# Onetism/LightFieldMicroscopy_PC-bzip2

Measured on AMD Instinct MI355X. Metric: uint16 Mpixel/s encode (predictor->bzip2) at 1/2/4/8 GPUs; ratio parity, higher is better.
Workload: dtype u16

## Files before the change

### lightfieldmicroscopy_pc-bzip2_amd/csrc/lfm_bzip2.hip

```cpp
#include <hip/hip_runtime.h>
#include <rocprim/block/block_exchange.hpp>
#include <rocprim/block/block_sort.hpp>
#include <rocprim/device/device_radix_sort.hpp>
#include <rocprim/device/device_scan.hpp>
#include <rocprim/device/device_segmented_radix_sort.hpp>
#include <rocprim/device/device_select.hpp>
#include <rocprim/iterator/counting_iterator.hpp>
#include <algorithm>
#include <climits>
#include <cstdlib>
#include <cstdint>
#include <cstdio>
#include <cstring>
#include <mutex>
#include <type_traits>
#include <vector>
#include "lfm_bwt_types.h"
#include "lfm_bz_caps.h"
#include "lfm_hip.h"
#include "lfm_huff_heap.h"

#ifndef LFM_BWT_FORCE_FULL
#define LFM_BWT_FORCE_FULL 0
#endif

namespace lfm {
namespace bz {

constexpr int kRleThreads = 512;
constexpr int kMaxGroups = 6;
constexpr int kMaxAlpha = 258;
constexpr int kIters = 4;
constexpr uint32_t kRunA = 0, kRunB = 1;

constexpr uint32_t kFlagHost = 1;

struct Geometry {
    uint32_t dims[5];
    uint32_t bs[5];
    uint32_t nb[5];
    uint32_t bpp;
};

struct Batch {
    const uint8_t* img;
    Geometry g;
    uint32_t first_block;
    uint32_t nstreams;
    uint32_t raw_cap;
    uint32_t cap;
    uint32_t level;
    uint32_t nblock_max;
    uint32_t out_cap;
    uint8_t* raw;
    uint32_t* raw_len;
    uint8_t* T;
    uint32_t* n;
    uint32_t* crc;
    uint32_t* inuse;
    uint32_t* flags;
    uint32_t* done;
    uint64_t* keys_a;
    uint64_t* keys_b;
    uint32_t* vals_a;
    uint32_t* sa;
    uint32_t* rank;
    uint32_t* vals_b;
    uint32_t* cl0;
    uint32_t* cl1;
    uint8_t* uflag;
    uint32_t* seg_begin;
    uint32_t* seg_end;
    uint16_t* mtfv;
// ... 2390 lines not shown
                pos += nz ? 1u : 0u;
                z = nz ? 0u : z + 1u;
            }
        }
        {
            uint32_t dsum = 0;
            for (uint64_t r = R; r; r &= r - 1ull) {
                const uint32_t i = (uint32_t)__builtin_ctzll(r), z = run_len(i);
                digits(wr + (uint32_t)__popcll(NZ & ((1ull << i) - 1ull)) + dsum, z);
                dsum += run_digits(z);
            }
        }
        if (has_last) {
            if (zend) digits(wr + w - 1u - dend, zend);
            tile_out[rle2_swz(wr + w - 1u)] = (uint16_t)EOB;
            atomicAdd(&freq[EOB], 1u);
        }
        __syncthreads();
        const uint32_t base = s_wr;
        for (uint32_t i = t; i < tile_total; i += kRle2Threads) out[base + i] = tile_out[rle2_swz(i)];
        __syncthreads();
        if (t == 0) {
            s_wr = base + tile_total;
            s_carry = tile_end_zeros;
        }
        __syncthreads();
    }
    static_assert(kRunA == 0 && kRunB == 1, "RUNA / RUNB are symbols 0 and 1");
    uint32_t cnts[6] = {nrunA, nrunB, (uint32_t)(hot & 0xFFFFu), (uint32_t)((hot >> 16) & 0xFFFFu),
                        (uint32_t)((hot >> 32) & 0xFFFFu), (uint32_t)(hot >> 48)};
#pragma unroll
    for (int r = 0; r < 6; ++r) {
        uint32_t c = cnts[r];
        for (int d = 32; d > 0; d >>= 1) c += (uint32_t)__shfl_xor((int)c, d);
        if (lane == 0 && c) atomicAdd(&freq[r], c);
    }
    __syncthreads();
    if (t == 0) {
        B.nmtf[s] = s_wr;
        if (!heap_narrow(B, s, (int)nin + 2)) B.wide[atomicAdd(B.wide_cnt, 1u)] = s;
    }
    for (uint32_t v = t; v < kMaxAlpha; v += kRle2Threads) B.mtf_freq[(size_t)s * kMaxAlpha + v] = freq[v];
}

constexpr int kHuffThreads = 256;

__device__ __forceinline__ uint32_t stream_nin(const Batch& B, uint32_t s)
{
    uint32_t nin = 0;
    for (int q = 0; q < 8; ++q) nin += __popc(B.inuse[s * 8 + q]);
    return nin;
}

__global__ __launch_bounds__(64) void huff_init(Batch B)
{
    __shared__ int mf[kMaxAlpha];
    __shared__ int pgs[kMaxGroups], pge[kMaxGroups];
    const uint32_t s = blockIdx.x, t = threadIdx.x;
    if (B.flags[s] & kFlagHost) return;
    const uint32_t nMTF = B.nmtf[s];
    const int alphaSize = (int)stream_nin(B, s) + 2;
    const uint32_t* mfreq = B.mtf_freq + (size_t)s * kMaxAlpha;
    uint8_t* len = B.len + (size_t)s * kMaxGroups * kMaxAlpha;
    const int nGroups = nMTF < 200 ? 2 : nMTF < 600 ? 3 : nMTF < 1200 ? 4 : nMTF < 2400 ? 5 : 6;
    for (int v = t; v < kMaxAlpha; v += 64) mf[v] = v < alphaSize ? (int)mfreq[v] : 0;
    __syncthreads();
    if (t == 0) {
        int nPart = nGroups, remF = (int)nMTF, gs = 0;
        while (nPart > 0) {
            const int tFreq = remF / nPart;
            int ge = gs - 1, aFreq = 0;
            while (aFreq < tFreq && ge < alphaSize - 1) {
                ++ge;
                aFreq += mf[ge];
            }
            if (ge > gs && nPart != nGroups && nPart != 1 && ((nGroups - nPart) % 2 == 1)) {
                aFreq -= mf[ge];
                --ge;
            }
            pgs[nPart - 1] = gs;
            pge[nPart - 1] = ge;
            --nPart;
            gs = ge + 1;
            remF -= aFreq;
        }
        B.ngroups[s] = (uint32_t)nGroups;
        B.nsel[s] = (nMTF + kGSize - 1) / kGSize;
    }
    __syncthreads();
    for (int i = t; i < kMaxGroups * kMaxAlpha; i += 64) {
        const int q = i / kMaxAlpha, v = i - q * kMaxAlpha;
        len[i] = (q < nGroups && v < alphaSize && v >= pgs[q] && v <= pge[q]) ? 0 : 15;
    }
}

__global__ __launch_bounds__(kHuffThreads) void huff_select_reg(Batch B)
{
    __shared__ uint32_t rfreq[kMaxGroups][kMaxAlpha];
    __shared__ uint64_t lpack[kMaxAlpha + 1];
    __shared__ uint32_t junk[kHuffThreads];
    const uint32_t s = blockIdx.x, t = threadIdx.x;
    if (B.flags[s] & kFlagHost) return;
    const uint32_t nMTF = B.nmtf[s], nSel = B.nsel[s];
    const int nGroups = (int)B.ngroups[s];
    const int alphaSize = (int)stream_nin(B, s) + 2;
    const uint8_t* len = B.len + (size_t)s * kMaxGroups * kMaxAlpha;
    const uint16_t* mtfv = B.mtfv + (size_t)s * (B.cap + 8);
    uint8_t* sel = B.sel + (size_t)s * B.sel_cap;
    for (int i = t; i < kMaxGroups * kMaxAlpha; i += kHuffThreads) rfreq[i / kMaxAlpha][i % kMaxAlpha] = 0;
    for (int v = t; v <= kMaxAlpha; v += kHuffThreads) {
        uint64_t lp = 0;
        if (v < alphaSize)
            for (int q = 0; q < nGroups; ++q) lp |= (uint64_t)len[q * kMaxAlpha + v] << (10 * q);
        lpack[v] = lp;
    }
    __syncthreads();
    uint64_t lp_hot[4];
#pragma unroll
    for (int f = 0; f < 4; ++f) lp_hot[f] = lpack[f];
    for (uint32_t g = t; g < nSel; g += kHuffThreads) {
        const uint32_t gs = g * kGSize, cnt = min(nMTF - gs, (uint32_t)kGSize);
        uint32_t w[kGSize / 2];
        if (cnt == (uint32_t)kGSize) {
            const uint32_t* p = (const uint32_t*)(mtfv + gs);
#pragma unroll
            for (int q = 0; q < kGSize / 2; ++q) w[q] = p[q];
        } else {
#pragma unroll
            for (int q = 0; q < kGSize / 2; ++q) {
                const uint32_t lo = 2u * q < cnt ? mtfv[gs + 2 * q] : (uint32_t)kMaxAlpha;
                const uint32_t hi = 2u * q + 1 < cnt ? mtfv[gs + 2 * q + 1] : (uint32_t)kMaxAlpha;
                w[q] = lo | (hi << 16);
            }
        }
        uint32_t hot = 0;
        uint64_t acc = 0;
#pragma unroll
        for (int q = 0; q < kGSize / 2; ++q) {
            const uint32_t lo = w[q] & 0xFFFFu, hi = w[q] >> 16;
            hot += lo < 4u ? 1u << (8u * lo) : 0u;
            hot += hi < 4u ? 1u << (8u * hi) : 0u;
            acc += lpack[lo < 4u ? (uint32_t)kMaxAlpha : lo] + lpack[hi < 4u ? (uint32_t)kMaxAlpha : hi];
        }
#pragma unroll
        for (uint32_t f = 0; f < 4; ++f) acc += (uint64_t)((hot >> (8u * f)) & 0xFFu) * lp_hot[f];
        int bt = -1;
        uint32_t bc = 999999999u;
        for (int q = 0; q < nGroups; ++q) {
            const uint32_t cq = (uint32_t)(acc >> (10 * q)) & 1023u;
            if (cq < bc) { bc = cq; bt = q; }
        }
        sel[g] = (uint8_t)bt;
#pragma unroll
        for (int q = 0; q < kGSize / 2; ++q) {
            const uint32_t lo = w[q] & 0xFFFFu, hi = w[q] >> 16;
            atomicAdd(lo >= 4u && lo != (uint32_t)kMaxAlpha ? &rfreq[bt][lo] : &junk[t], 1u);
            atomicAdd(hi >= 4u && hi != (uint32_t)kMaxAlpha ? &rfreq[bt][hi] : &junk[t], 1u);
        }
#pragma unroll
        for (uint32_t f = 0; f < 4; ++f)
            if ((hot >> (8u * f)) & 0xFFu) atomicAdd(&rfreq[bt][f], (hot >> (8u * f)) & 0xFFu);
    }
    __syncthreads();
    uint32_t* rf = B.rfreq + (size_t)s * kMaxGroups * kMaxAlpha;
    for (int i = t; i < kMaxGroups * kMaxAlpha; i += kHuffThreads) rf[i] = rfreq[i / kMaxAlpha][i % kMaxAlpha];
}

template <typename Ent, int kL>
struct LdsHeap {
    static constexpr uint32_t RS = sizeof(Ent) * kL;
    char* base;
    uint16_t* parent;
    __device__ __forceinline__ Ent ld(uint32_t e) const { return *(const Ent*)(base + e * RS); }
    __device__ __forceinline__ void st(uint32_t e, Ent v) const { *(Ent*)(base + e * RS) = v; }
    __device__ __forceinline__ void ld_pair(uint32_t e, Ent& a, Ent& b) const
    {
        const char* q = base + e * RS;
        a = *(const Ent*)q;
        b = *(const Ent*)(q + RS);
    }
    __device__ __forceinline__ void fence() const { __builtin_amdgcn_sched_barrier(0); }
    __device__ __forceinline__ void set_parent(uint32_t node, uint32_t p) const { parent[node] = (uint16_t)p; }
    __device__ __forceinline__ bool any(bool b) const { return __builtin_amdgcn_ballot_w64(b) != 0; }
    __device__ __forceinline__ void note_sift(uint32_t, uint32_t) const {}
    __device__ __forceinline__ void note_push(uint32_t, uint32_t) const {}
    __device__ __forceinline__ void check(const HeapPref&, uint32_t) const {}
};

template <typename Ent>
constexpr int kHeapMaxRetries = sizeof(Ent) == 4 ? 17 : 32;

template <typename Ent, int kL>
__device__ __forceinline__ void heap_code_lengths(const Batch& B, char* hb, uint32_t lane, uint32_t s, uint32_t tb)
{
    constexpr uint32_t ES = sizeof(Ent);
    static_assert(kHeapEntries * sizeof(Ent) * kL <= 33792, "the heaps' LDS grew");
    static_assert(kHeapEntries >= kMaxAlpha + 2 && 2 * kMaxAlpha / (int)(ES / 2) < kHeapEntries, "heap entries");
    {
        const int A = (int)stream_nin(B, s) + 2;
        const uint32_t* freq = B.rfreq + ((size_t)s * kMaxGroups + tb) * kMaxAlpha;
        uint8_t* len = B.len + ((size_t)s * kMaxGroups + tb) * kMaxAlpha;
        uint16_t* parent = (uint16_t*)(B.code + ((size_t)s * kMaxGroups + tb) * kMaxAlpha);
        LdsHeap<Ent, kL> acc{hb + lane * ES, parent};
        auto ent = [&](uint32_t e) -> Ent& { return *(Ent*)(acc.base + e * LdsHeap<Ent, kL>::RS); };
        auto dep = [&](uint32_t k) -> uint16_t& {
            return *(uint16_t*)((char*)&ent(k / (ES / 2)) + 2 * (k % (ES / 2)));
        };
        auto ld2 = [](const void* p, int i) { return *(const uint2*)((const uint32_t*)p + (i > 0 ? i : 0)); };
        constexpr Ent kSent = ~(Ent)0;
        auto upheap_init = [&](uint32_t z) {
            constexpr int D = 9;
            Ent v[D + 1];
#pragma unroll
            for (int j = 0; j <= D; ++j) v[j] = ent(z >> j);
            __builtin_amdgcn_sched_barrier(0);
            const Ent k = v[0], kk = k | (Ent)1023;
            bool below = true;
#pragma unroll
            for (int j = 0; j < D; ++j) {
                const bool lt = kk < v[j + 1];
                ent(z >> j) = lt ? v[j + 1] : (below || j == 0 ? k : v[j]);
                below = lt;
            }
        };
        int retries = 0;
        uint32_t nMerged = (uint32_t)A;
        bool build = true;
        for (int round = 0; round <= kHeapMaxRetries<Ent>; ++round) {
            uint32_t nHeap = 1, tooLong = 0;
            Ent top = 0;
            HeapPref m;
            if (build) {
                ent(0) = 0;
                for (int e = A + 1; e < kHeapEntries; ++e) ent((uint32_t)e) = kSent;
                for (int i0 = 1; i0 <= A; i0 += 32) {
                    uint2 f[16];
#pragma unroll
                    for (int q = 0; q < 16; ++q) f[q] = ld2(freq, min(i0 - 1 + 2 * q, kMaxAlpha - 2));
#pragma unroll
                    for (int q = 0; q < 16; ++q) {
                        const int i = i0 + 2 * q;
                        uint32_t w0 = f[q].x ? f[q].x : 1u, w1 = f[q].y ? f[q].y : 1u;
                        for (int r = 0; r < retries; ++r) {
                            w0 = 1u + w0 / 2u;
                            w1 = 1u + w1 / 2u;
                        }
                        if (i <= A) ent(i) = ((Ent)w0 << 15) | (Ent)i;
                        if (i + 1 <= A) ent(i + 1) = ((Ent)w1 << 15) | (Ent)(i + 1);
                    }
                }
                for (int i = 1; i <= A; ++i) upheap_init((uint32_t)i);
                heap_pref_build<Ent>(acc, m, (uint32_t)A);
                nHeap = (uint32_t)A;
                nMerged = (uint32_t)A;
                top = ent(1);
            }
            uint32_t hmax = 0;
            for (int b = 8; b >= 0; --b) {
                const uint32_t a = build ? (uint32_t)A : 0u;
                if (__builtin_amdgcn_ballot_w64((a >> b & 1u) && (a >> (b + 1)) == (hmax >> (b + 1)))) hmax |= 1u << b;
            }
            hmax = min(__builtin_amdgcn_readfirstlane(hmax), (uint32_t)kMaxAlpha);
            for (; hmax > 1u; --hmax)
                if (build && nHeap > 1u) heap_merge_step_at<Ent>(acc, m, hmax, nHeap, nMerged, top, tooLong);
            build = build && tooLong && retries < kHeapMaxRetries<Ent>;
            if (build) ++retries;
            if (!__builtin_amdgcn_ballot_w64(build)) break;
        }
        const int nNodes = (int)nMerged;
        if (retries) atomicAdd(B.wide_cnt + 1, (uint32_t)retries);
        dep(nNodes) = 0;
        for (int kc = (nNodes - 1) & ~63; kc >= 0; kc -= 64) {
            uint2 pw[16];
#pragma unroll
            for (int q = 0; q < 16; ++q) pw[q] = ld2(parent, min(kc / 2 + 2 * q, (2 * kMaxAlpha) / 2 - 2));
#pragma unroll
            for (int q = 15; q >= 0; --q) {
                const int b = kc + 4 * q;
                const uint32_t p4[4] = {pw[q].x & 0xFFFFu, pw[q].x >> 16, pw[q].y & 0xFFFFu, pw[q].y >> 16};
                uint32_t d[4], dn[4];
#pragma unroll
                for (int r = 0; r < 4; ++r) d[r] = dep(min(p4[r], 2u * kMaxAlpha));
#pragma unroll
                for (int r = 3; r >= 0; --r) {
                    const int k = b + r;
                    uint32_t x = d[r];
#pragma unroll
                    for (int u = r + 1; u < 4; ++u) x = p4[r] == (uint32_t)(b + u) ? dn[u] : x;
                    dn[r] = k == nNodes ? 0u : x + 1u;
                    if (k >= 1 && k < nNodes) dep(k) = (uint16_t)dn[r];
                }
            }
        }
        for (int i = 1; i <= A; ++i) len[i - 1] = (uint8_t)dep(i);
    }
}

template <int kL>
__global__ __launch_bounds__(64) void huff_lengths_heap(Batch B, uint32_t nwg_wide, uint32_t nwide_streams)
{
    __shared__ uint32_t hq[kHeapEntries * kL];
    char* hb = (char*)hq;
    const uint32_t lane = threadIdx.x;
    if (blockIdx.x >= nwg_wide) {
        const uint32_t task = (blockIdx.x - nwg_wide) * kL + lane;
        const uint32_t s = task / kMaxGroups, tb = task % kMaxGroups;
        if (lane >= (uint32_t)kL || s >= B.nstreams || (B.flags[s] & kFlagHost) || tb >= B.ngroups[s]) return;
        if (!heap_narrow(B, s, (int)stream_nin(B, s) + 2)) return;
        heap_code_lengths<uint32_t, kL>(B, hb, lane, s, tb);
    } else {
        constexpr int kW = kL / 2;
        const uint32_t i = blockIdx.x * kW + lane;
        if (lane >= (uint32_t)kW || i >= nwide_streams * kMaxGroups) return;
        const uint32_t s = B.wide[i / kMaxGroups], tb = i % kMaxGroups;
        if ((B.flags[s] & kFlagHost) || tb >= B.ngroups[s]) return;
        heap_code_lengths<uint64_t, kW>(B, hb, lane, s, tb);
    }
}

__global__ __launch_bounds__(64) void huff_final(Batch B)
{
    const uint32_t s = blockIdx.x, lane = threadIdx.x;
    if (B.flags[s] & kFlagHost) return;
    const uint32_t nGroups = B.ngroups[s];
    const uint32_t nSel = B.nsel[s];
    const uint32_t alphaSize = stream_nin(B, s) + 2;
    const uint8_t* len = B.len + (size_t)s * kMaxGroups * kMaxAlpha;
    {
        const uint8_t* sel = B.sel + (size_t)s * B.sel_cap;
        uint8_t* sm = B.sel_mtf + (size_t)s * B.sel_cap;
        uint32_t pos = 0x543210u;
        for (uint32_t i0 = 0; i0 < nSel; i0 += 64) {
            const uint32_t cnt = min(64u, nSel - i0);
            const uint32_t v = lane < cnt ? sel[i0 + lane] : 0u;
            uint32_t out = 0;
            for (uint32_t g = 0; g < cnt; ++g) {
                const uint32_t ll = __builtin_amdgcn_readlane(v, g);
                const uint32_t x = pos ^ (ll * 0x111111u);
                const uint32_t z = (x - 0x111111u) & ~x & 0x888888u;
                const uint32_t j = (uint32_t)__builtin_ctz(z) >> 2;
                const uint32_t m = (1u << (4 * (j + 1))) - 1u;
                pos = (pos & ~m) | (((pos << 4) | ll) & m);
                out = lane == g ? j : out;
            }
            if (lane < cnt) sm[i0 + lane] = (uint8_t)out;
        }
    }
    const uint64_t lt = (1ull << lane) - 1ull;
    for (uint32_t q = 0; q < nGroups; ++q) {
        const uint8_t* lq = len + q * kMaxAlpha;
        uint32_t* code = B.code + ((size_t)s * kMaxGroups + q) * kMaxAlpha;
        uint32_t L[5], c[5];
#pragma unroll
        for (int k = 0; k < 5; ++k) {
            const uint32_t i = 64 * k + lane;
            L[k] = i < alphaSize ? lq[i] : 0u;
            c[k] = 0;
        }
        uint32_t vec = 0;
        for (uint32_t nl = 1; nl <= 20; ++nl) {
            uint32_t before = 0;
#pragma unroll
            for (int k = 0; k < 5; ++k) {
                const uint64_t b = __ballot(L[k] == nl);
                if (L[k] == nl) c[k] = vec + before + (uint32_t)__popcll(b & lt);
                before += (uint32_t)__popcll(b);
            }
            vec = (vec + before) << 1;
        }
#pragma unroll
        for (int k = 0; k < 5; ++k) {
            const uint32_t i = 64 * k + lane;
            if (i < alphaSize) code[i] = c[k];
        }
    }
}

constexpr int kEmitThreads = 256;

__device__ __forceinline__ void put_bits_atomic(uint32_t* words, uint64_t pos, uint32_t nbits, uint32_t v)
{
    if (!nbits) return;
    const uint32_t w = (uint32_t)(pos >> 5), o = (uint32_t)(pos & 31);
    const uint64_t sh = ((uint64_t)v << (64 - nbits)) >> o;
    const uint32_t hi = (uint32_t)(sh >> 32), lo = (uint32_t)sh;
    if (hi) atomicOr(&words[w], hi);
    if (lo) atomicOr(&words[w + 1], lo);
}

constexpr uint32_t kSelLds = 8192;

constexpr uint32_t kHdrWords = 4096;

__device__ __forceinline__ void put_bits_hdr(uint32_t* hdr, uint32_t* words, uint64_t pos, uint32_t nbits, uint32_t v)
{
    if (!nbits) return;
    const uint32_t w = (uint32_t)(pos >> 5), o = (uint32_t)(pos & 31);
    const uint64_t sh = ((uint64_t)v << (64 - nbits)) >> o;
    const uint32_t hi = (uint32_t)(sh >> 32), lo = (uint32_t)sh;
    if (w + 1 < kHdrWords) {
        hdr[w] |= hi;
        hdr[w + 1] |= lo;
    } else {
        if (hi) atomicOr(&words[w], hi);
        if (lo) atomicOr(&words[w + 1], lo);
    }
}

__device__ __forceinline__ void put_bits_hdr_atomic(uint32_t* hdr, uint32_t* words, uint64_t pos, uint32_t nbits,
                                                    uint32_t v)
{
    if (!nbits) return;
    const uint32_t w = (uint32_t)(pos >> 5), o = (uint32_t)(pos & 31);
    const uint64_t sh = ((uint64_t)v << (64 - nbits)) >> o;
    const uint32_t hi = (uint32_t)(sh >> 32), lo = (uint32_t)sh;
    if (w + 1 < kHdrWords) {
        if (hi) atomicOr(&hdr[w], hi);
        if (lo) atomicOr(&hdr[w + 1], lo);
    } else {
        if (hi) atomicOr(&words[w], hi);
        if (lo) atomicOr(&words[w + 1], lo);
    }
}

__device__ __forceinline__ void put_bits64_hdr_atomic(uint32_t* hdr, uint32_t* words, uint64_t pos, uint32_t nbits,
                                                      uint64_t v)
{
    if (nbits > 32) {
// ... 825 lines not shown
extern "C" size_t lfm_hip_bzip2_workspace_bytes_multi(uint32_t nstreams, uint32_t block_bytes, uint32_t level)
{
    if (level < 1 || level > 9) return 0;
    Batch B{};
    Scratch S{};
    return layout(nullptr, nstreams, block_bytes, level, B, S);
}

extern "C" uint32_t lfm_hip_bzip2_max_count_multi(uint32_t block_bytes, uint32_t level)
{
    if (level < 1 || level > 9) return 0;
    Batch B{};
    Scratch S{};
    (void)layout(nullptr, 0, block_bytes, level, B, S);
    return (uint32_t)(((1ull << 32) - 1) / ((uint64_t)B.parts * B.cap));
}

extern "C" size_t lfm_hip_bzip2_out_cap(uint32_t block_bytes) { return out_cap(block_bytes); }

namespace {
int bzip2_blocks(const void* d_img, const uint32_t dims[5], const uint32_t bs[5], uint32_t bpp, uint32_t first,
                 const uint32_t streams, uint32_t level, void* d_ws, size_t ws_bytes, void* d_payload,
                 uint64_t* h_sizes, uint32_t* h_flags, void* stream_, bool multi)
{
    uint32_t count = streams;
    hipStream_t st = (hipStream_t)stream_;
    if (!d_img || !dims || !bs || !bpp || !count || level < 1 || level > 9 || !d_ws || !d_payload) return LFM_HIP_EINVAL;
    int dev = 0;
    (void)hipGetDevice(&dev);
    if (!crc_tables_on_device(dev)) return LFM_HIP_ERUNTIME;
    StageEvents& SE = t_stage;
    SE.valid = false;
    const bool timed = SE.ready(dev);
    auto mark = [&](int i) {
        if (timed) (void)hipEventRecord(SE.ev[i], st);
    };
    Batch B{};
    B.img = (const uint8_t*)d_img;
    uint32_t raw_cap = bpp;
    for (int d = 0; d < 5; ++d) {
        B.g.dims[d] = dims[d];
        B.g.bs[d] = bs[d];
        B.g.nb[d] = (uint32_t)((dims[d] + bs[d] - 1) / bs[d]);
        raw_cap *= bs[d];
    }
    B.g.bpp = bpp;
    B.first_block = first;
    B.level = level;
    B.nblock_max = 100000u * level - 19u;
    Scratch S{};
    if (ws_bytes < layout((uint8_t*)d_ws, streams, raw_cap, multi ? level : 0u, B, S)) return LFM_HIP_EINVAL;
    count = B.nstreams;
    if ((size_t)count * B.cap >= (1ull << 32)) return LFM_HIP_EINVAL;
    const bool parts = B.parts > 1;

    hipError_t e = hipSuccess;
    auto ok = [&]() { return (e = hipGetLastError()) == hipSuccess; };
    const bool from_img = ((uintptr_t)d_img & 15) == 0 && (bs[0] * bpp) % 16 == 0 && (dims[0] * bpp) % 16 == 0 &&
                          ((dims[0] % bs[0]) * bpp) % 16 == 0;
    mark(0);
    if (!from_img) hipLaunchKernelGGL(gather_blocks, dim3(64, streams), dim3(256), 0, st, B);
    if (!parts) {
        if (from_img) hipLaunchKernelGGL((rle1_crc<true, false>), dim3(count), dim3(kRleThreads), 0, st, B);
        else hipLaunchKernelGGL((rle1_crc<false, false>), dim3(count), dim3(kRleThreads), 0, st, B);
    } else {
        if (from_img) hipLaunchKernelGGL((rle1_crc<true, true>), dim3(streams), dim3(kRleThreads), 0, st, B);
        else hipLaunchKernelGGL((rle1_crc<false, true>), dim3(streams), dim3(kRleThreads), 0, st, B);
        hipLaunchKernelGGL(place_parts, dim3(16, count), dim3(256), 0, st, B);
    }
    if (!ok()) return LFM_HIP_ERUNTIME;
    mark(1);
    BwtStats bwt_stats;
    B.ent = (uint2*)B.keys_a;
    if (bwt_sort(B, S, st, &bwt_stats) != hipSuccess) return LFM_HIP_ERUNTIME;
    t_last_place = bwt_stats.place_path(B.it_full != 0);
    {
        const uint32_t v[12] = {bwt_stats.chunks[0], bwt_stats.chunks[1], bwt_stats.chunks[2], bwt_stats.chunks[3],
                                bwt_stats.first_ties, bwt_stats.left_runs, bwt_stats.text_rounds, bwt_stats.restarted,
                                bwt_stats.rank_form, bwt_stats.doubling_rounds, bwt_stats.flag_periodic, 0u};
        std::copy(v, v + 12, t_last_bwt);
        std::copy(bwt_stats.jobs, bwt_stats.jobs + 4, t_last_jobs);
    }
    if (!B.it_full) {
        const uint32_t chunks = (B.cap + kPlaceChunk - 1) / kPlaceChunk;
        if (t_last_place == 2)
            hipLaunchKernelGGL(bwt_place_sorted, dim3(8 * chunks * ((count + 7) / 8)), dim3(256), 0, st, B, chunks);
        hipLaunchKernelGGL(bwt_induce, dim3(count), dim3(64), 0, st, B);
        if (!ok()) return LFM_HIP_ERUNTIME;
    }
    mark(2);
    if (t_hook) t_hook(t_hook_ctx, 1);
    {
        const uint32_t nseg_max = (B.cap + kSeg - 1) / kSeg;
        int32_t* seg_last = (int32_t*)B.keys_a;
        const dim3 g((nseg_max + 3) / 4, count);
        if (B.it_full) hipLaunchKernelGGL(mtf_last<false>, g, dim3(256), 0, st, B, nseg_max, seg_last);
        else hipLaunchKernelGGL(mtf_last<true>, g, dim3(256), 0, st, B, nseg_max, seg_last);
        hipLaunchKernelGGL(mtf_prefix, dim3(count), dim3(256), 0, st, B, nseg_max, seg_last);
        hipLaunchKernelGGL(mtf_win, g, dim3(256), 0, st, B, nseg_max, (const int32_t*)seg_last);
        hipLaunchKernelGGL(rle2, dim3(count), dim3(kRle2Threads), 0, st, B);
    }
    uint32_t nwide = 0;
    if (!ok() || hipMemcpyAsync(&nwide, B.wide_cnt, 4, hipMemcpyDeviceToHost, st) != hipSuccess ||
        hipStreamSynchronize(st) != hipSuccess || nwide > count)
        return LFM_HIP_ERUNTIME;
    mark(3);
    if (t_hook) t_hook(t_hook_ctx, 2);
    hipLaunchKernelGGL(huff_init, dim3(count), dim3(64), 0, st, B);
    static thread_local struct TablesEvent {
        hipEvent_t ev = nullptr;
        int dev = -1;
        ~TablesEvent()
        {
            if (ev) (void)hipEventDestroy(ev);
        }
    } tables_ev;
    if (t_hook && tables_ev.dev != dev) {
        if (tables_ev.ev) (void)hipEventDestroy(tables_ev.ev);
        tables_ev.ev = nullptr;
        tables_ev.dev = -1;
        if (hipEventCreateWithFlags(&tables_ev.ev, hipEventDisableTiming) == hipSuccess) tables_ev.dev = dev;
    }
    hipEvent_t ev_tables = tables_ev.ev;
    for (int it = 0; it < kIters; ++it) {
        hipLaunchKernelGGL(huff_select_reg, dim3(count), dim3(kHuffThreads), 0, st, B);
        constexpr uint32_t kPlane = 32;
        const uint32_t nn = (count * kMaxGroups + kPlane - 1) / kPlane;
        const uint32_t nw = (nwide * kMaxGroups + kPlane / 2 - 1) / (kPlane / 2);
        hipLaunchKernelGGL(huff_lengths_heap<kPlane>, dim3(nn + nw), dim3(64), 0, st, B, nw, nwide);
    }
    hipLaunchKernelGGL(huff_final, dim3(count), dim3(64), 0, st, B);
    mark(4);
    const bool hook3 = t_hook && ev_tables && hipEventRecord(ev_tables, st) == hipSuccess;
    Batch J = B;
    if (!parts) {
        hipLaunchKernelGGL(emit_stream<false>, dim3(count), dim3(kEmitThreads), 0, st, B);
    } else {
        hipLaunchKernelGGL(emit_stream<true>, dim3(count), dim3(kEmitThreads), 0, st, B);
        hipLaunchKernelGGL(join_parts, dim3(streams), dim3(256), 0, st, B);
        J.words = B.jwords;
        J.out_cap = B.jcap;
        J.out_bytes = B.sbytes;
        J.flags = B.sflags;
    }
    hipLaunchKernelGGL(scan_offsets, dim3(1), dim3(1024), 0, st, J.out_bytes, streams, S.offs);
    hipLaunchKernelGGL(compact_streams, dim3(streams), dim3(256), 0, st, J, S.offs, (uint8_t*)d_payload);
    mark(5);
    if (!ok()) return LFM_HIP_ERUNTIME;
    if (hook3 && hipEventSynchronize(ev_tables) == hipSuccess) t_hook(t_hook_ctx, 3);
    static const bool stats = std::getenv("LFM_BZ2_STATS") && std::atoi(std::getenv("LFM_BZ2_STATS")) != 0;
    if (stats) {
        uint32_t c[8] = {};
        if (hipMemcpyAsync(c, S.cnt, 32, hipMemcpyDeviceToHost, st) == hipSuccess && hipStreamSynchronize(st) == hipSuccess)
            std::fprintf(stderr, "lfm_bzip2 stats: %u streams, %u with u64 Huffman heaps, Huffman retries %u, "
                         "tied after the chunk sorts %u, runs left to the tie rounds %u\n", count, c[3], c[4],
                         bwt_stats.first_ties, bwt_stats.left_runs);
    }
    std::vector<uint32_t> nbytes(streams), np(streams, 1u);
    if (hipMemcpyAsync(nbytes.data(), J.out_bytes, streams * 4, hipMemcpyDeviceToHost, st) != hipSuccess ||
        hipMemcpyAsync(h_flags, J.flags, streams * 4, hipMemcpyDeviceToHost, st) != hipSuccess ||
        (parts && hipMemcpyAsync(np.data(), B.nparts, streams * 4, hipMemcpyDeviceToHost, st) != hipSuccess) ||
        hipStreamSynchronize(st) != hipSuccess)
        return LFM_HIP_ERUNTIME;
    for (uint32_t i = 0; i < streams; ++i) h_sizes[i] = nbytes[i];
    t_last_blocks = 0;
    for (uint32_t i = 0; i < streams; ++i) t_last_blocks += h_flags[i] ? 0u : np[i];
    if (timed) {
        SE.valid = true;
        for (int i = 0; i < 5; ++i)
            if (hipEventElapsedTime(&SE.last_ms[i], SE.ev[i], SE.ev[i + 1]) != hipSuccess) SE.valid = false;
    }
    return LFM_HIP_OK;
}
}

extern "C" int lfm_hip_bzip2_blocks(const void* d_img, const uint32_t dims[5], const uint32_t bs[5], uint32_t bpp,
                                    uint32_t first, uint32_t count, uint32_t level, void* d_ws, size_t ws_bytes,
                                    void* d_payload, uint64_t* h_sizes, uint32_t* h_flags, void* stream)
{
    return bzip2_blocks(d_img, dims, bs, bpp, first, count, level, d_ws, ws_bytes, d_payload, h_sizes, h_flags, stream,
                        false);
}

extern "C" int lfm_hip_bzip2_blocks_multi(const void* d_img, const uint32_t dims[5], const uint32_t bs[5],
                                          uint32_t bpp, uint32_t first, uint32_t count, uint32_t level, void* d_ws,
                                          size_t ws_bytes, void* d_payload, uint64_t* h_sizes, uint32_t* h_flags,
                                          void* stream)
{
    return bzip2_blocks(d_img, dims, bs, bpp, first, count, level, d_ws, ws_bytes, d_payload, h_sizes, h_flags, stream,
                        true);
}

extern "C" void lfm_hip_bzip2_set_stage_hook(void (*fn)(void*, int), void* ctx)
{
    t_hook = fn;
    t_hook_ctx = ctx;
}

extern "C" uint64_t lfm_hip_bzip2_last_blocks(void) { return t_last_blocks; }

extern "C" void lfm_hip_bzip2_last_bwt_stats(uint32_t out[12])
{
    if (out) std::copy(t_last_bwt, t_last_bwt + 12, out);
}

extern "C" void lfm_hip_bzip2_last_sort_jobs(uint32_t out[4])
{
    if (out) std::copy(t_last_jobs, t_last_jobs + 4, out);
}

extern "C" uint32_t lfm_hip_bzip2_last_place_path(void) { return t_last_place; }

extern "C" int lfm_hip_bzip2_last_stage_ms(float ms[5])
{
    if (!ms || !t_stage.valid) return 3;
    for (int i = 0; i < 5; ++i) ms[i] = t_stage.last_ms[i];
    return 0;
}
```

### lightfieldmicroscopy_pc-bzip2_amd/csrc/lfm_huff_heap.h

```cpp
#pragma once
#include <cstdint>

#ifndef LFM_HD
#if defined(__HIPCC__) || defined(__CUDACC__)
#define LFM_HD __host__ __device__
#else
#define LFM_HD
#endif
#endif

constexpr int kHeapEntries = 264;
constexpr uint32_t kHeapSentPair = 260;
constexpr int kHeapMaxLevels = 8;
constexpr int kPrefWords = 5;

struct HeapPref {
    uint32_t w[kPrefWords];
};

template <typename Ent>
LFM_HD inline bool heap_wless(Ent a, Ent b)
{
    return (a | (Ent)1023) < b;
}

template <typename Ent>
LFM_HD inline Ent heap_sent()
{
    return ~(Ent)0;
}

LFM_HD inline uint32_t heap_pref_at(const HeapPref& m, int j, uint32_t p)
{
    if (j <= 4) return (m.w[0] >> (p & 31u)) & 1u;
    if (j == 5) return (m.w[1] >> (p & 31u)) & 1u;
    if (j == 6) return ((p & 32u ? m.w[3] : m.w[2]) >> (p & 31u)) & 1u;
    const uint32_t b = p - 128u < 31u ? p - 128u : 31u;
    return (m.w[4] >> b) & 1u;
}

LFM_HD inline uint32_t heap_put_bit(uint32_t w, uint32_t b, uint32_t bit)
{
    return (w & ~(1u << b)) | (bit << b);
}

LFM_HD inline void heap_pref_flip(HeapPref& d, int j, uint32_t p, uint32_t flip)
{
    if (j <= 4) {
        d.w[0] |= flip << (p & 31u);
    } else if (j == 5) {
        d.w[1] |= flip << (p & 31u);
    } else if (j == 6) {
        const uint32_t x = flip << (p & 31u);
        d.w[2] |= p & 32u ? 0u : x;
        d.w[3] |= p & 32u ? x : 0u;
    } else {
        const uint32_t b = p - 128u < 31u ? p - 128u : 31u;
        d.w[4] |= flip << b;
    }
}

LFM_HD inline void heap_pref_set_any(HeapPref& m, uint32_t p, uint32_t bit)
{
    const uint32_t b = p & 31u, wi = p >> 5;
#pragma unroll
    for (uint32_t i = 0; i < (uint32_t)kPrefWords; ++i) m.w[i] = wi == i ? heap_put_bit(m.w[i], b, bit) : m.w[i];
}

template <typename Ent, typename Acc>
LFM_HD inline void heap_pref_build(Acc& acc, HeapPref& m, uint32_t A)
{
    const uint32_t last = A >> 1;
#pragma unroll
    for (uint32_t wi = 0; wi < (uint32_t)kPrefWords; ++wi) {
        uint32_t word = 0;
        for (uint32_t b0 = 0; b0 < 32u && 32u * wi + b0 <= last; b0 += 8u) {
            Ent l[8], r[8];
#pragma unroll
            for (uint32_t q = 0; q < 8u; ++q) {
                const uint32_t p = 32u * wi + b0 + q;
                acc.ld_pair(2u * (p <= last ? p : last), l[q], r[q]);
            }
            acc.fence();
#pragma unroll
            for (uint32_t q = 0; q < 8u; ++q) {
                const uint32_t p = 32u * wi + b0 + q;
                word |= (p >= 1u && p <= last && heap_wless(r[q], l[q]) ? 1u : 0u) << (b0 + q);
            }
        }
        m.w[wi] = word;
    }
}

template <int L, typename Ent, typename Acc>
LFM_HD inline Ent heap_sift_path(Acc& acc, HeapPref& m, Ent k)
{
    if constexpr (L == 0) {
        acc.st(1u, k);
        acc.note_sift(0u, 0u);
        return k;
    } else {
        uint32_t p[L + 1], cb[L], r[L];
        p[0] = 1u;
#pragma unroll
        for (int j = 0; j < L; ++j) {
            r[j] = heap_pref_at(m, j, p[j]);
            cb[j] = 2u * p[j];
            if (j == 7) cb[j] = cb[j] < kHeapSentPair ? cb[j] : kHeapSentPair;
            p[j + 1] = cb[j] | r[j];
        }
        Ent a[L], b[L];
#pragma unroll
        for (int j = 0; j < L; ++j) acc.ld_pair(cb[j], a[j], b[j]);
        acc.fence();
        const Ent kk = k | (Ent)1023;
        Ent c[L], sib[L], nv[L + 1];
        bool go[L];
        bool g = true;
        uint32_t went = 0;
#pragma unroll
        for (int j = 0; j < L; ++j) {
// ... 135 lines not shown
```

Before: 19000.

## Parallelize selector MTF scan, fold huff_init into first select pass, split huff_final waves

Replaces the serial per-selector MTF loop in huff_final with a wave-wide parallel prefix scan over MTF-list summaries, and runs it in a dedicated wave alongside per-group code-assignment waves. huff_init is removed, and its partitioning is folded into a templated first huff_select_reg pass, which saves a launch and a global round-trip of the length table. Heap initial build is restructured into level-templated inserts, and optional timestamp instrumentation is added. This adds composition work per lane and requires 16-byte alignment of selector buffers.

```diff
diff --git a/lightfieldmicroscopy_pc-bzip2_amd/csrc/lfm_bzip2.hip b/lightfieldmicroscopy_pc-bzip2_amd/csrc/lfm_bzip2.hip
--- a/lightfieldmicroscopy_pc-bzip2_amd/csrc/lfm_bzip2.hip
+++ b/lightfieldmicroscopy_pc-bzip2_amd/csrc/lfm_bzip2.hip
@@ -19,6 +19,7 @@
 #include "lfm_bz_caps.h"
 #include "lfm_hip.h"
 #include "lfm_huff_heap.h"
+#include "lfm_sel_mtf.h"
 
 #ifndef LFM_BWT_FORCE_FULL
 #define LFM_BWT_FORCE_FULL 0
@@ -2515,18 +2516,11 @@
     return nin;
 }
 
-__global__ __launch_bounds__(64) void huff_init(Batch B)
-{
-    __shared__ int mf[kMaxAlpha];
-    __shared__ int pgs[kMaxGroups], pge[kMaxGroups];
-    const uint32_t s = blockIdx.x, t = threadIdx.x;
-    if (B.flags[s] & kFlagHost) return;
-    const uint32_t nMTF = B.nmtf[s];
-    const int alphaSize = (int)stream_nin(B, s) + 2;
+__device__ __forceinline__ void huff_partition(const Batch& B, uint32_t s, uint32_t t, uint32_t nthreads, uint32_t nMTF,
+                                               int alphaSize, int nGroups, int* mf, int* pgs, int* pge)
+{
     const uint32_t* mfreq = B.mtf_freq + (size_t)s * kMaxAlpha;
-    uint8_t* len = B.len + (size_t)s * kMaxGroups * kMaxAlpha;
-    const int nGroups = nMTF < 200 ? 2 : nMTF < 600 ? 3 : nMTF < 1200 ? 4 : nMTF < 2400 ? 5 : 6;
-    for (int v = t; v < kMaxAlpha; v += 64) mf[v] = v < alphaSize ? (int)mfreq[v] : 0;
+    for (int v = t; v < kMaxAlpha; v += nthreads) mf[v] = v < alphaSize ? (int)mfreq[v] : 0;
     __syncthreads();
     if (t == 0) {
         int nPart = nGroups, remF = (int)nMTF, gs = 0;
@@ -2551,32 +2545,37 @@
         B.nsel[s] = (nMTF + kGSize - 1) / kGSize;
     }
     __syncthreads();
-    for (int i = t; i < kMaxGroups * kMaxAlpha; i += 64) {
-        const int q = i / kMaxAlpha, v = i - q * kMaxAlpha;
-        len[i] = (q < nGroups && v < alphaSize && v >= pgs[q] && v <= pge[q]) ? 0 : 15;
-    }
-}
-
+}
+
+template <bool FIRST>
 __global__ __launch_bounds__(kHuffThreads) void huff_select_reg(Batch B)
 {
     __shared__ uint32_t rfreq[kMaxGroups][kMaxAlpha];
     __shared__ uint64_t lpack[kMaxAlpha + 1];
     __shared__ uint32_t junk[kHuffThreads];
+    __shared__ int pgs[kMaxGroups], pge[kMaxGroups];
     const uint32_t s = blockIdx.x, t = threadIdx.x;
     if (B.flags[s] & kFlagHost) return;
-    const uint32_t nMTF = B.nmtf[s], nSel = B.nsel[s];
-    const int nGroups = (int)B.ngroups[s];
+    const uint32_t nMTF = B.nmtf[s];
+    const uint32_t nSel = FIRST ? (nMTF + kGSize - 1) / kGSize : B.nsel[s];
+    int nGroups;
+    if constexpr (FIRST) nGroups = nMTF < 200 ? 2 : nMTF < 600 ? 3 : nMTF < 1200 ? 4 : nMTF < 2400 ? 5 : 6;
+    else nGroups = (int)B.ngroups[s];
     const int alphaSize = (int)stream_nin(B, s) + 2;
     const uint8_t* len = B.len + (size_t)s * kMaxGroups * kMaxAlpha;
     const uint16_t* mtfv = B.mtfv + (size_t)s * (B.cap + 8);
     uint8_t* sel = B.sel + (size_t)s * B.sel_cap;
-    for (int i = t; i < kMaxGroups * kMaxAlpha; i += kHuffThreads) rfreq[i / kMaxAlpha][i % kMaxAlpha] = 0;
+    if constexpr (FIRST) huff_partition(B, s, t, kHuffThreads, nMTF, alphaSize, nGroups, (int*)&rfreq[0][0], pgs, pge);
     for (int v = t; v <= kMaxAlpha; v += kHuffThreads) {
         uint64_t lp = 0;
         if (v < alphaSize)
-            for (int q = 0; q < nGroups; ++q) lp |= (uint64_t)len[q * kMaxAlpha + v] << (10 * q);
+            for (int q = 0; q < nGroups; ++q) {
+                const uint32_t l = FIRST ? (v >= pgs[q] && v <= pge[q] ? 0u : 15u) : (uint32_t)len[q * kMaxAlpha + v];
+                lp |= (uint64_t)l << (10 * q);
+            }
         lpack[v] = lp;
     }
+    for (int i = t; i < kMaxGroups * kMaxAlpha; i += kHuffThreads) rfreq[i / kMaxAlpha][i % kMaxAlpha] = 0;
     __syncthreads();
     uint64_t lp_hot[4];
 #pragma unroll
@@ -2628,6 +2627,37 @@
     uint32_t* rf = B.rfreq + (size_t)s * kMaxGroups * kMaxAlpha;
     for (int i = t; i < kMaxGroups * kMaxAlpha; i += kHuffThreads) rf[i] = rfreq[i / kMaxAlpha][i % kMaxAlpha];
 }
+
+
+#ifdef LFM_HUFF_STAMPS
+constexpr uint32_t kStampWgs = 4096, kStampSlots = 8;
+__device__ unsigned long long g_huff_stamps[2][kStampWgs][kStampSlots];
+struct HuffStamps {
+    unsigned long long last, d[kStampSlots];
+    __device__ __forceinline__ void start()
+    {
+        for (uint32_t p = 0; p < kStampSlots; ++p) d[p] = 0;
+        __builtin_amdgcn_sched_barrier(0);
+        last = __builtin_amdgcn_s_memtime();
+    }
+    __device__ __forceinline__ void mark(uint32_t p)
+    {
+        __builtin_amdgcn_sched_barrier(0);
+        const unsigned long long now = __builtin_amdgcn_s_memtime();
+        __builtin_amdgcn_sched_barrier(0);
+        d[p] += now - last;
+        last = now;
+    }
+    __device__ __forceinline__ void store(uint32_t row, uint32_t p0, uint32_t np) const
+    {
+        if (blockIdx.x < kStampWgs)
+            for (uint32_t p = p0; p < p0 + np; ++p) atomicMax(&g_huff_stamps[row][blockIdx.x][p], d[p]);
+    }
+};
+#define HUFF_STAMPS(x) x
+#else
+#define HUFF_STAMPS(x)
+#endif
 
 template <typename Ent, int kL>
 struct LdsHeap {
@@ -2671,24 +2701,11 @@
         };
         auto ld2 = [](const void* p, int i) { return *(const uint2*)((const uint32_t*)p + (i > 0 ? i : 0)); };
         constexpr Ent kSent = ~(Ent)0;
-        auto upheap_init = [&](uint32_t z) {
-            constexpr int D = 9;
-            Ent v[D + 1];
-#pragma unroll
-            for (int j = 0; j <= D; ++j) v[j] = ent(z >> j);
-            __builtin_amdgcn_sched_barrier(0);
-            const Ent k = v[0], kk = k | (Ent)1023;
-            bool below = true;
-#pragma unroll
-            for (int j = 0; j < D; ++j) {
-                const bool lt = kk < v[j + 1];
-                ent(z >> j) = lt ? v[j + 1] : (below || j == 0 ? k : v[j]);
-                below = lt;
-            }
-        };
+        constexpr int kLoads = 16;
         int retries = 0;
         uint32_t nMerged = (uint32_t)A;
         bool build = true;
+        HUFF_STAMPS(HuffStamps ts; ts.start();)
         for (int round = 0; round <= kHeapMaxRetries<Ent>; ++round) {
             uint32_t nHeap = 1, tooLong = 0;
             Ent top = 0;
@@ -2696,12 +2713,12 @@
             if (build) {
                 ent(0) = 0;
                 for (int e = A + 1; e < kHeapEntries; ++e) ent((uint32_t)e) = kSent;
-                for (int i0 = 1; i0 <= A; i0 += 32) {
-                    uint2 f[16];
-#pragma unroll
-                    for (int q = 0; q < 16; ++q) f[q] = ld2(freq, min(i0 - 1 + 2 * q, kMaxAlpha - 2));
-#pragma unroll
-                    for (int q = 0; q < 16; ++q) {
+                for (int i0 = 1; i0 <= A; i0 += 2 * kLoads) {
+                    uint2 f[kLoads];
+#pragma unroll
+                    for (int q = 0; q < kLoads; ++q) f[q] = ld2(freq, min(i0 - 1 + 2 * q, kMaxAlpha - 2));
+#pragma unroll
+                    for (int q = 0; q < kLoads; ++q) {
                         const int i = i0 + 2 * q;
                         uint32_t w0 = f[q].x ? f[q].x : 1u, w1 = f[q].y ? f[q].y : 1u;
                         for (int r = 0; r < retries; ++r) {
@@ -2712,8 +2729,11 @@
                         if (i + 1 <= A) ent(i + 1) = ((Ent)w1 << 15) | (Ent)(i + 1);
                     }
                 }
-                for (int i = 1; i <= A; ++i) upheap_init((uint32_t)i);
+                HUFF_STAMPS(ts.mark(0);)
+                heap_insert_levels<Ent>(acc, (uint32_t)A);
+                HUFF_STAMPS(ts.mark(1);)
                 heap_pref_build<Ent>(acc, m, (uint32_t)A);
+                HUFF_STAMPS(ts.mark(2);)
                 nHeap = (uint32_t)A;
                 nMerged = (uint32_t)A;
                 top = ent(1);
@@ -2726,6 +2746,7 @@
             hmax = min(__builtin_amdgcn_readfirstlane(hmax), (uint32_t)kMaxAlpha);
             for (; hmax > 1u; --hmax)
                 if (build && nHeap > 1u) heap_merge_step_at<Ent>(acc, m, hmax, nHeap, nMerged, top, tooLong);
+            HUFF_STAMPS(ts.mark(3);)
             build = build && tooLong && retries < kHeapMaxRetries<Ent>;
             if (build) ++retries;
             if (!__builtin_amdgcn_ballot_w64(build)) break;
@@ -2733,12 +2754,12 @@
         const int nNodes = (int)nMerged;
         if (retries) atomicAdd(B.wide_cnt + 1, (uint32_t)retries);
         dep(nNodes) = 0;
-        for (int kc = (nNodes - 1) & ~63; kc >= 0; kc -= 64) {
-            uint2 pw[16];
-#pragma unroll
-            for (int q = 0; q < 16; ++q) pw[q] = ld2(parent, min(kc / 2 + 2 * q, (2 * kMaxAlpha) / 2 - 2));
-#pragma unroll
-            for (int q = 15; q >= 0; --q) {
+        for (int kc = (nNodes - 1) & ~(4 * kLoads - 1); kc >= 0; kc -= 4 * kLoads) {
+            uint2 pw[kLoads];
+#pragma unroll
+            for (int q = 0; q < kLoads; ++q) pw[q] = ld2(parent, min(kc / 2 + 2 * q, (2 * kMaxAlpha) / 2 - 2));
+#pragma unroll
+            for (int q = kLoads - 1; q >= 0; --q) {
                 const int b = kc + 4 * q;
                 const uint32_t p4[4] = {pw[q].x & 0xFFFFu, pw[q].x >> 16, pw[q].y & 0xFFFFu, pw[q].y >> 16};
                 uint32_t d[4], dn[4];
@@ -2755,7 +2776,9 @@
                 }
             }
         }
+        HUFF_STAMPS(ts.mark(4);)
         for (int i = 1; i <= A; ++i) len[i - 1] = (uint8_t)dep(i);
+        HUFF_STAMPS(ts.mark(5); ts.store(0, 0, 6);)
     }
 }
 
@@ -2781,36 +2804,65 @@
     }
 }
 
-__global__ __launch_bounds__(64) void huff_final(Batch B)
-{
-    const uint32_t s = blockIdx.x, lane = threadIdx.x;
+constexpr uint32_t kSelChunk = 32;
+constexpr uint32_t kFinalWaves = kMaxGroups + 1;
+static_assert(kSelChunk % 16 == 0, "a lane's chunk is loaded and stored in 16-byte pieces");
+
+__device__ __forceinline__ void sel_mtf_scan(const uint8_t* __restrict__ sel, uint8_t* __restrict__ sm, uint32_t nSel,
+                                             uint32_t lane)
+{
+    constexpr uint32_t NQ = kSelChunk / 16;
+    uint32_t carry = kSelMtfStart;
+    for (uint32_t i0 = 0; i0 < nSel; i0 += kSelMtfLanes * kSelChunk) {
+        const uint32_t b = i0 + lane * kSelChunk;
+        const uint32_t n = selmtf_chunk_count(nSel, i0, lane, kSelChunk);
+        uint32_t w[4 * NQ];
+#pragma unroll
+        for (uint32_t q = 0; q < NQ; ++q) {
+            uint4 v = make_uint4(0u, 0u, 0u, 0u);
+            if (b + 16u * q < nSel) v = *(const uint4*)(sel + b + 16u * q);
+            w[4 * q] = v.x, w[4 * q + 1] = v.y, w[4 * q + 2] = v.z, w[4 * q + 3] = v.w;
+        }
+        auto get = [&](uint32_t g) { return (w[g >> 2] >> (8u * (g & 3u))) & 0xFFu; };
+        uint32_t incl = selmtf_summary(get, n, kSelChunk);
+        if (lane == 0) incl = selmtf_compose(carry, incl);
+#pragma unroll
+        for (uint32_t d = 1; d < kSelMtfLanes; d <<= 1) {
+            const uint32_t prev = (uint32_t)__shfl_up((int)incl, d);
+            const uint32_t both = selmtf_compose(prev, incl);
+            incl = lane >= d ? both : incl;
+        }
+        const uint32_t before = (uint32_t)__shfl_up((int)incl, 1);
+        uint32_t o[4 * NQ];
+#pragma unroll
+        for (uint32_t q = 0; q < 4 * NQ; ++q) o[q] = 0;
+        selmtf_replay(lane ? before : carry, get, [&](uint32_t g, uint32_t j) { o[g >> 2] |= j << (8u * (g & 3u)); }, n,
+                      kSelChunk);
+#pragma unroll
+        for (uint32_t q = 0; q < NQ; ++q)
+            if (b + 16u * q < nSel) *(uint4*)(sm + b + 16u * q) = make_uint4(o[4 * q], o[4 * q + 1], o[4 * q + 2], o[4 * q + 3]);
+        carry = (uint32_t)__builtin_amdgcn_readlane((int)incl, kSelMtfLanes - 1);
+    }
+}
+
+__global__ __launch_bounds__(64 * kFinalWaves) void huff_final(Batch B)
+{
+    const uint32_t s = blockIdx.x, lane = threadIdx.x & 63u;
+    const uint32_t wave = __builtin_amdgcn_readfirstlane(threadIdx.x >> 6);
     if (B.flags[s] & kFlagHost) return;
     const uint32_t nGroups = B.ngroups[s];
-    const uint32_t nSel = B.nsel[s];
+    HUFF_STAMPS(HuffStamps ts; ts.start();)
+    if (wave == (uint32_t)kMaxGroups) {
+        sel_mtf_scan(B.sel + (size_t)s * B.sel_cap, B.sel_mtf + (size_t)s * B.sel_cap, B.nsel[s], lane);
+        HUFF_STAMPS(ts.mark(0); ts.store(1, 0, 1);)
+        return;
+    }
+    if (wave >= nGroups) return;
     const uint32_t alphaSize = stream_nin(B, s) + 2;
     const uint8_t* len = B.len + (size_t)s * kMaxGroups * kMaxAlpha;
+    const uint64_t lt = (1ull << lane) - 1ull;
     {
-        const uint8_t* sel = B.sel + (size_t)s * B.sel_cap;
-        uint8_t* sm = B.sel_mtf + (size_t)s * B.sel_cap;
-        uint32_t pos = 0x543210u;
-        for (uint32_t i0 = 0; i0 < nSel; i0 += 64) {
-            const uint32_t cnt = min(64u, nSel - i0);
-            const uint32_t v = lane < cnt ? sel[i0 + lane] : 0u;
-            uint32_t out = 0;
-            for (uint32_t g = 0; g < cnt; ++g) {
-                const uint32_t ll = __builtin_amdgcn_readlane(v, g);
-                const uint32_t x = pos ^ (ll * 0x111111u);
-                const uint32_t z = (x - 0x111111u) & ~x & 0x888888u;
-                const uint32_t j = (uint32_t)__builtin_ctz(z) >> 2;
-                const uint32_t m = (1u << (4 * (j + 1))) - 1u;
-                pos = (pos & ~m) | (((pos << 4) | ll) & m);
-                out = lane == g ? j : out;
-            }
-            if (lane < cnt) sm[i0 + lane] = (uint8_t)out;
-        }
-    }
-    const uint64_t lt = (1ull << lane) - 1ull;
-    for (uint32_t q = 0; q < nGroups; ++q) {
+        const uint32_t q = wave;
         const uint8_t* lq = len + q * kMaxAlpha;
         uint32_t* code = B.code + ((size_t)s * kMaxGroups + q) * kMaxAlpha;
         uint32_t L[5], c[5];
@@ -2837,6 +2889,7 @@
             if (i < alphaSize) code[i] = c[k];
         }
     }
+    HUFF_STAMPS(ts.mark(1); if (wave == 0) ts.store(1, 1, 1);)
 }
 
 constexpr int kEmitThreads = 256;
@@ -3768,6 +3821,7 @@
     if (ws_bytes < layout((uint8_t*)d_ws, streams, raw_cap, multi ? level : 0u, B, S)) return LFM_HIP_EINVAL;
     count = B.nstreams;
     if ((size_t)count * B.cap >= (1ull << 32)) return LFM_HIP_EINVAL;
+    if (B.sel_cap % 16 || ((uintptr_t)d_ws & 15)) return LFM_HIP_EINVAL;
     const bool parts = B.parts > 1;
 
     hipError_t e = hipSuccess;
@@ -3822,7 +3876,6 @@
         return LFM_HIP_ERUNTIME;
     mark(3);
     if (t_hook) t_hook(t_hook_ctx, 2);
-    hipLaunchKernelGGL(huff_init, dim3(count), dim3(64), 0, st, B);
     static thread_local struct TablesEvent {
         hipEvent_t ev = nullptr;
         int dev = -1;
@@ -3839,13 +3892,14 @@
     }
     hipEvent_t ev_tables = tables_ev.ev;
     for (int it = 0; it < kIters; ++it) {
-        hipLaunchKernelGGL(huff_select_reg, dim3(count), dim3(kHuffThreads), 0, st, B);
+        if (it == 0) hipLaunchKernelGGL(huff_select_reg<true>, dim3(count), dim3(kHuffThreads), 0, st, B);
+        else hipLaunchKernelGGL(huff_select_reg<false>, dim3(count), dim3(kHuffThreads), 0, st, B);
         constexpr uint32_t kPlane = 32;
         const uint32_t nn = (count * kMaxGroups + kPlane - 1) / kPlane;
         const uint32_t nw = (nwide * kMaxGroups + kPlane / 2 - 1) / (kPlane / 2);
         hipLaunchKernelGGL(huff_lengths_heap<kPlane>, dim3(nn + nw), dim3(64), 0, st, B, nw, nwide);
     }
-    hipLaunchKernelGGL(huff_final, dim3(count), dim3(64), 0, st, B);
+    hipLaunchKernelGGL(huff_final, dim3(count), dim3(64 * kFinalWaves), 0, st, B);
     mark(4);
     const bool hook3 = t_hook && ev_tables && hipEventRecord(ev_tables, st) == hipSuccess;
     Batch J = B;
@@ -3933,3 +3987,15 @@
     for (int i = 0; i < 5; ++i) ms[i] = t_stage.last_ms[i];
     return 0;
 }
+
+#ifdef LFM_HUFF_STAMPS
+extern "C" int lfm_hip_huff_stamps(unsigned long long* out)
+{
+    if (!out || hipDeviceSynchronize() != hipSuccess) return 3;
+    const size_t bytes = sizeof(unsigned long long) * 2 * kStampWgs * kStampSlots;
+    void* d = nullptr;
+    if (hipGetSymbolAddress(&d, HIP_SYMBOL(g_huff_stamps)) != hipSuccess) return 3;
+    if (hipMemcpy(out, d, bytes, hipMemcpyDeviceToHost) != hipSuccess || hipMemset(d, 0, bytes) != hipSuccess) return 3;
+    return 0;
+}
+#endif
diff --git a/lightfieldmicroscopy_pc-bzip2_amd/csrc/lfm_huff_heap.h b/lightfieldmicroscopy_pc-bzip2_amd/csrc/lfm_huff_heap.h
--- a/lightfieldmicroscopy_pc-bzip2_amd/csrc/lfm_huff_heap.h
+++ b/lightfieldmicroscopy_pc-bzip2_amd/csrc/lfm_huff_heap.h
@@ -67,6 +67,44 @@
     for (uint32_t i = 0; i < (uint32_t)kPrefWords; ++i) m.w[i] = wi == i ? heap_put_bit(m.w[i], b, bit) : m.w[i];
 }
 
+template <int J, typename Ent, typename Acc>
+LFM_HD inline void heap_insert_at(Acc& acc, uint32_t z)
+{
+    Ent v[J + 1];
+#pragma unroll
+    for (int j = 0; j <= J; ++j) v[j] = acc.ld(z >> j);
+    acc.fence();
+    const Ent k = v[0], kk = k | (Ent)1023;
+    bool below = true;
+#pragma unroll
+    for (int j = 0; j < J; ++j) {
+        const bool lt = kk < v[j + 1];
+        acc.st(z >> j, lt ? v[j + 1] : (below ? k : v[j]));
+        below = lt;
+    }
+    acc.st(1u, below ? k : v[J]);
+}
+
+template <int J, typename Ent, typename Acc>
+LFM_HD inline void heap_insert_level(Acc& acc, uint32_t A)
+{
+    const uint32_t last = A < (2u << J) - 1u ? A : (2u << J) - 1u;
+    for (uint32_t z = 1u << J; z <= last; ++z) heap_insert_at<J, Ent>(acc, z);
+}
+
+template <typename Ent, typename Acc>
+LFM_HD inline void heap_insert_levels(Acc& acc, uint32_t A)
+{
+    heap_insert_level<1, Ent>(acc, A);
+    heap_insert_level<2, Ent>(acc, A);
+    heap_insert_level<3, Ent>(acc, A);
+    heap_insert_level<4, Ent>(acc, A);
+    heap_insert_level<5, Ent>(acc, A);
+    heap_insert_level<6, Ent>(acc, A);
+    heap_insert_level<7, Ent>(acc, A);
+    heap_insert_level<8, Ent>(acc, A);
+}
+
 template <typename Ent, typename Acc>
 LFM_HD inline void heap_pref_build(Acc& acc, HeapPref& m, uint32_t A)
 {
diff --git a/lightfieldmicroscopy_pc-bzip2_amd/csrc/lfm_sel_mtf.h b/lightfieldmicroscopy_pc-bzip2_amd/csrc/lfm_sel_mtf.h
--- /dev/null
+++ b/lightfieldmicroscopy_pc-bzip2_amd/csrc/lfm_sel_mtf.h
@@ -0,0 +1,132 @@
+#pragma once
+#include <cstdint>
+
+#ifndef LFM_HD
+#if defined(__HIPCC__) || defined(__CUDACC__)
+#define LFM_HD __host__ __device__
+#else
+#define LFM_HD
+#endif
+#endif
+
+constexpr uint32_t kSelMtfStart = 0x543210u;
+constexpr uint32_t kSelMtfEmpty = 0xFFFFFFu;
+constexpr uint32_t kSelMtfLanes = 64;
+
+LFM_HD inline uint32_t selmtf_zero_nibbles(uint32_t x)
+{
+    return (x - 0x111111u) & ~x & 0x888888u;
+}
+
+LFM_HD inline uint32_t selmtf_front(uint32_t list, uint32_t j, uint32_t ll)
+{
+    const uint32_t m = (1u << (4u * (j + 1u))) - 1u;
+    return (list & ~m) | (((list << 4) | ll) & m);
+}
+
+LFM_HD inline uint32_t selmtf_step(uint32_t& list, uint32_t ll)
+{
+    const uint32_t z = selmtf_zero_nibbles(list ^ (ll * 0x111111u)) | 0x800000u;
+    const uint32_t j = (uint32_t)__builtin_ctz(z) >> 2;
+    list = selmtf_front(list, j, ll);
+    return j;
+}
+
+LFM_HD inline void selmtf_step_any(uint32_t& list, uint32_t ll)
+{
+    const uint32_t z = selmtf_zero_nibbles(list ^ (ll * 0x111111u)) | selmtf_zero_nibbles(~list & 0xFFFFFFu) | 0x800000u;
+    list = selmtf_front(list, (uint32_t)__builtin_ctz(z) >> 2, ll);
+}
+
+LFM_HD inline uint32_t selmtf_count(uint32_t summary)
+{
+    uint32_t n = 0;
+#pragma unroll
+    for (uint32_t i = 0; i < 6u; ++i) n += ((summary >> (4u * i)) & 15u) != 15u ? 1u : 0u;
+    return n;
+}
+
+template <typename Get>
+LFM_HD inline uint32_t selmtf_summary(Get get, uint32_t n, uint32_t C)
+{
+    uint32_t list = kSelMtfEmpty;
+#pragma unroll
+    for (uint32_t g = 0; g < C; ++g) {
+        uint32_t next = list;
+        selmtf_step_any(next, get(g) & 7u);
+        list = g < n ? next : list;
+    }
+    return list;
+}
+
+LFM_HD inline uint32_t selmtf_compose(uint32_t earlier, uint32_t later)
+{
+    uint32_t list = earlier;
+#pragma unroll
+    for (int i = 5; i >= 0; --i) {
+        const uint32_t ll = (later >> (4 * i)) & 15u;
+        uint32_t next = list;
+        selmtf_step_any(next, ll);
+        list = ll != 15u ? next : list;
+    }
+    return list;
+}
+
+template <typename Get, typename Put>
+LFM_HD inline uint32_t selmtf_replay(uint32_t list, Get get, Put put, uint32_t n, uint32_t C)
+{
+#pragma unroll
+    for (uint32_t g = 0; g < C; ++g) {
+        uint32_t next = list;
+        const uint32_t j = selmtf_step(next, get(g) & 7u);
+        list = g < n ? next : list;
+        put(g, g < n ? j : 0u);
+    }
+    return list;
+}
+
+LFM_HD inline uint32_t selmtf_chunk_count(uint32_t nSel, uint32_t i0, uint32_t lane, uint32_t C)
+{
+    const uint32_t b = i0 + lane * C;
+    return b >= nSel ? 0u : (nSel - b < C ? nSel - b : C);
+}
+
+#if !defined(__HIP_DEVICE_COMPILE__)
+struct SelMtfMet {
+    uint64_t passes_with_carry = 0, chunks_of_six = 0, chunks_of_one = 0;
+};
+
+inline void selmtf_scan_host(const uint8_t* sel, uint8_t* out, uint32_t nSel, uint32_t C, SelMtfMet* met = nullptr,
+                             uint32_t lanes = kSelMtfLanes)
+{
+    uint32_t carry = kSelMtfStart;
+    for (uint32_t i0 = 0; i0 < nSel; i0 += lanes * C) {
+        uint32_t incl[kSelMtfLanes], n[kSelMtfLanes];
+        for (uint32_t l = 0; l < lanes; ++l) {
+            n[l] = selmtf_chunk_count(nSel, i0, l, C);
+            const uint8_t* p = sel + i0 + l * C;
+            const uint32_t nl = n[l];
+            const uint32_t sum = selmtf_summary([&](uint32_t g) { return g < nl ? (uint32_t)p[g] : 7u; }, nl, C);
+            if (met) {
+                met->chunks_of_six += selmtf_count(sum) == 6u;
+                met->chunks_of_one += nl >= 2u && selmtf_count(sum) == 1u;
+            }
+            incl[l] = l == 0 ? selmtf_compose(carry, sum) : sum;
+        }
+        if (met && i0) ++met->passes_with_carry;
+        for (uint32_t d = 1; d < lanes; d <<= 1) {
+            uint32_t prev[kSelMtfLanes];
+            for (uint32_t l = 0; l < lanes; ++l) prev[l] = l >= d ? incl[l - d] : 0u;
+            for (uint32_t l = d; l < lanes; ++l) incl[l] = selmtf_compose(prev[l], incl[l]);
+        }
+        for (uint32_t l = 0; l < lanes; ++l) {
+            const uint8_t* p = sel + i0 + l * C;
+            uint8_t* o = out + i0 + l * C;
+            const uint32_t nl = n[l];
+            selmtf_replay(l ? incl[l - 1] : carry, [&](uint32_t g) { return g < nl ? (uint32_t)p[g] : 7u; },
+                          [&](uint32_t g, uint32_t j) { if (g < nl) o[g] = (uint8_t)j; }, nl, C);
+        }
+        carry = incl[lanes - 1];
+    }
+}
+#endif
```

After: 19460, median of 6. 2.4% higher.
